# keeffEoghan/tendrils

Measured on AMD Instinct MI355X. Metric: particle-steps/sec (16M particles per GPU), higher is better.
Workload: dtype f32

## Files before the change

tendrils_amd/csrc/th_api.hip:

```cpp
#include "th_ctx.hpp"

using namespace thi;

namespace {

thread_local std::string g_error;

void build_gradient_table(float4 *lut)
{
    for (int a = th::kLutMin; a <= th::kLutMax; ++a) {
        float p = th::permute_ref((float)a);
        float gx, gy, gz;
        th::gradient_ref(p, gx, gy, gz);
        lut[a - th::kLutMin] = make_float4(gx, gy, gz, 0.0f);
    }
}

void options_from_environment(th_options &o)
{
    auto number = [](const char *name, long long otherwise) { const char *e = getenv(name); return e && *e ? atoll(e) : otherwise; };
    o.bucket = (int)number("TH_BUCKET", -1);
    o.resort_steps = (int)number("TH_RESORT_STEPS", 64); if (o.resort_steps <= 0) o.resort_steps = 64;
    o.rebucket_steps = (int)number("TH_REBUCKET_STEPS", 256); if (o.rebucket_steps <= 0) o.rebucket_steps = 256;
    o.fuse = number("TH_FUSE", 1) != 0;
// ... 111 lines not shown

}

extern "C" {

int32_t th_abi_version(void) { return TH_ABI_VERSION; }

const char *th_last_error(void) { return g_error.c_str(); }

th_status th_device_count(int32_t *count)
{
    TH_REQUIRE(count, "null count");
    int n = 0;
    hipError_t e = hipGetDeviceCount(&n);
    if (e != hipSuccess) { *count = 0; return fail(TH_ERR_NO_DEVICE, "hipGetDeviceCount: %s", hipGetErrorString(e)); }
    *count = n;
    return TH_OK;
}

th_status th_create(const th_config *cfg, th_context **out)
{
    TH_REQUIRE(cfg && out, "null argument");
    *out = nullptr;
    TH_REQUIRE(cfg->width > 0 && cfg->height > 0, "state shape must be positive (got %dx%d)", cfg->width, cfg->height);
    TH_REQUIRE(cfg->num_buffers >= 0 && cfg->num_buffers <= 64, "num_buffers out of range");
    TH_REQUIRE(cfg->mode == TH_MODE_EXACT || cfg->mode == TH_MODE_FAST, "unknown mode %d", cfg->mode);
    TH_REQUIRE(cfg->state_format == TH_STATE_F32 || cfg->state_format == TH_STATE_F16, "unknown state format %d", cfg->state_format);
    TH_REQUIRE((uint64_t)cfg->width * (uint64_t)cfg->height < (1ull << 31), "more than 2^31 texels per context");
    int n = 0;
    if (hipGetDeviceCount(&n) != hipSuccess || n <= 0) return fail(TH_ERR_NO_DEVICE, "no HIP device available");
    TH_REQUIRE(cfg->device >= 0 && cfg->device < n, "device %d out of range (have %d)", cfg->device, n);
    hipDeviceProp_t prop;
    TH_HIP(hipGetDeviceProperties(&prop, cfg->device));
    if (strncmp(prop.gcnArchName, "gfx950", 6) != 0)
        return fail(TH_ERR_NO_DEVICE, "device %d is %s; this library ships gfx950 code only", cfg->device, prop.gcnArchName);

    th_context *c = new (std::nothrow) th_context;
    if (!c) return fail(TH_ERR_INVALID, "out of host memory");
    c->cfg = *cfg;
    options_from_environment(c->opt);
    c->packed = cfg->state_format == TH_STATE_F16;
    if (c->cfg.global_height <= 0) c->cfg.global_height = c->cfg.height;
    if (c->cfg.row0 < 0 || c->cfg.row0 + c->cfg.height > c->cfg.global_height) {
        delete c;
        return fail(TH_ERR_INVALID, "row band [%d,%d) outside global height %d", cfg->row0, cfg->row0 + cfg->height, cfg->global_height);
    }
    th_status st = TH_OK;
    auto body = [&]() -> th_status {
        TH_HIP(hipSetDevice(c->cfg.device));
        TH_HIP(hipStreamCreateWithFlags(&c->stream, hipStreamNonBlocking));
        TH_HIP(hipEventCreate(&c->ev0));
        TH_HIP(hipEventCreate(&c->ev1));
        const size_t hv = (size_t)th::hash_table_vectors();
        TH_HIP(hipMalloc((void **)&c->lut_block, (hv + th::kLutSize) * sizeof(float4)));
        c->lut = c->lut_block + hv;
        std::vector<float4> lut(th::kLutSize);
        build_gradient_table(lut.data());
        TH_HIP(hipMemcpy(c->lut, lut.data(), lut.size() * sizeof(float4), hipMemcpyHostToDevice));
        th::launch_hash_tables(c->lut_block, c->stream);
        TH_HIP(hipGetLastError());
        TH_HIP(hipMalloc((void **)&c->d_flag, sizeof(unsigned int)));
        TH_HIP(hipMalloc((void **)&c->partials, th::kStatsBlocks * sizeof(th::StatsPartial)));
        TH_HIP(hipMalloc((void **)&c->d_counters, sizeof(th_counters)));
        TH_HIP(hipMalloc((void **)&c->d_respawned, 2 * sizeof(unsigned long long)));
        TH_HIP(hipMemset(c->d_respawned, 0, 2 * sizeof(unsigned long long)));
        c->fw = c->fh = 1;
        TH_HIP(hipMalloc((void **)&c->flow, sizeof(float4)));
        TH_HIP(hipMemsetAsync(c->flow, 0, sizeof(float4), c->stream));
        TH_HIP(hipMalloc((void **)&c->flow_dec, sizeof(float2)));
        TH_HIP(hipMalloc((void **)&c->targets, c->texels() * sizeof(float4)));
        TH_HIP(hipMemsetAsync(c->targets, 0, c->texels() * sizeof(float4), c->stream));
        for (int k = 0; k < c->cfg.num_buffers; ++k) {
            float4 *b = nullptr;
            if (th_status s = alloc_state(c, &b)) return s;
            c->ring.push_back(b);
        }
        if (th_status s = line_rows(c)) return s;
        TH_HIP(hipStreamSynchronize(c->stream));
        return TH_OK;
    };
    st = body();
    if (st != TH_OK) { std::string keep = g_error; th_destroy(c); g_error = keep; return st; }
    *out = c;
    return TH_OK;
}

th_status th_destroy(th_context *c)
{
    if (!c) return TH_OK;
    (void)hipSetDevice(c->cfg.device);
    if (c->stream) (void)hipStreamSynchronize(c->stream);
    if (c->side) (void)hipStreamSynchronize(c->side);
    if (c->side2) (void)hipStreamSynchronize(c->side2);
    if (c->comm) { (void)c->transport->destroy(c->comm); c->comm = nullptr; }
    (void)hipFree(c->d_status); (void)hipFree(c->own_mem);
    thi::flow_lines_free(c);
    for (float4 *b : c->ring) (void)hipFree(b);
    (void)hipFree(c->flow); (void)hipFree(c->flow_dec); (void)hipFree(c->flow3); (void)hipFree(c->targets); (void)hipFree(c->lut_block);
    (void)hipFree(c->frames[0]); (void)hipFree(c->frames[1]);
    (void)hipFree(c->dep_count); (void)hipFree(c->dep_offset); (void)hipFree(c->dep_blocks); (void)hipFree(c->dep_total);
    (void)hipFree(c->dep_record); (void)hipFree(c->dep_lists); (void)hipFree(c->mrg_keys2); (void)hipFree(c->mrg_colors);
    (void)hipFree(c->bin_mem); (void)hipFree(c->draw_blocks); (void)hipFree(c->draw_block_flags); (void)hipFree(c->d_row_draws); (void)hipFree(c->src_row_index); (void)hipFree(c->src_col_index); (void)hipFree(c->src_slots); (void)hipFree(c->edge_rows); (void)hipFree(c->crowd_mem); (void)hipFree(c->chunk_table);
    (void)hipFree(c->bins_keys); (void)hipFree(c->bins_colors); (void)hipFree(c->crowd_keys); (void)hipFree(c->crowd_sorted); (void)hipFree(c->crowd_parted); (void)hipFree(c->crowd_windows); (void)hipFree(c->gathered);
    if (c->forked) (void)hipEventDestroy(c->forked);
    if (c->joined) (void)hipEventDestroy(c->joined);
    if (c->side) (void)hipStreamDestroy(c->side);
    if (c->joined2) (void)hipEventDestroy(c->joined2);
// ... 397 lines not shown
```

tendrils_amd/csrc/th_kernels.hip:

```cpp
#include "th_kernels.hpp"
#include "th_math.hpp"
#include "th_logic.hpp"

#include <type_traits>
#include <cstdlib>

namespace th {


static int grid_for(size_t n, int blocks_per_cu)
{
    size_t blocks = (n + 255) / 256;
    size_t cap = (size_t)256 * blocks_per_cu;
    return (int)(blocks < cap ? (blocks ? blocks : 1) : cap);
}



__global__ __launch_bounds__(256) void pack_state_kernel(uint2 *dst, const float4 *src, uint32_t n)
{
    for (uint32_t i = blockIdx.x * 256u + threadIdx.x; i < n; i += gridDim.x * 256u) dst[i] = pack_state(src[i]);
}

__global__ __launch_bounds__(256) void unpack_state_kernel(float4 *dst, const uint2 *src, uint32_t n)
{
    for (uint32_t i = blockIdx.x * 256u + threadIdx.x; i < n; i += gridDim.x * 256u) dst[i] = unpack_state(src[i]);
}

void launch_pack_state(void *dst, const float4 *src, uint32_t n, hipStream_t s)
{
    if (n) hipLaunchKernelGGL(pack_state_kernel, dim3(grid_for(n, 8)), dim3(256), 0, s, (uint2 *)dst, src, n);
}

void launch_unpack_state(float4 *dst, const void *src, uint32_t n, hipStream_t s)
{
    if (n) hipLaunchKernelGGL(unpack_state_kernel, dim3(grid_for(n, 8)), dim3(256), 0, s, dst, (const uint2 *)src, n);
}

__global__ __launch_bounds__(256) void hash_tables_kernel(float4 *block)
{
    uint32_t *a = reinterpret_cast<uint32_t *>(block), *b = a + kPermA;
    for (int k = threadIdx.x; k < kPermA; k += 256) a[k] = 4u * (uint32_t)permute_int((float)k);
    for (int k = threadIdx.x; k < kPermB; k += 256) b[k] = 16u * (uint32_t)((int)permute_int((float)k) - kLutMin);
}
void launch_hash_tables(float4 *block, hipStream_t s) { hipLaunchKernelGGL(hash_tables_kernel, dim3(1), dim3(256), 0, s, block); }
int hash_table_vectors() { return kHashVec; }



struct F32Texel {
    using Word = float4;
    static constexpr bool packed = false;
    TH_D static Word empty() { return make_float4(0.0f, 0.0f, 0.0f, 0.0f); }
    TH_D static Word load(const float4 *buf, uint32_t i) { return load_stream(&buf[i]); }
    TH_D static void store(float4 *buf, uint32_t i, Word w) { store_stream(&buf[i], w); }
    TH_D static float4 decode(Word w) { return w; }
    TH_D static Word encode(float4 s) { return s; }
    TH_D static float4 quantize(float4 s) { return s; }
};
struct PackedTexel {
    using Word = v2u;
    static constexpr bool packed = true;
    TH_D static Word empty() { return Word{0x80008000u, 0u}; }
    TH_D static Word load(const float4 *buf, uint32_t i) { return __builtin_nontemporal_load(&reinterpret_cast<const v2u *>(buf)[i]); }
    TH_D static void store(float4 *buf, uint32_t i, Word w) { __builtin_nontemporal_store(w, &reinterpret_cast<v2u *>(buf)[i]); }
    TH_D static float4 decode(Word w) { return unpack_state(make_uint2(w.x, w.y)); }
    TH_D static Word encode(float4 s) { const uint2 q = pack_state(s); return Word{q.x, q.y}; }
    TH_D static float4 quantize(float4 s) { return quantize_state(s); }
};


#define TH_LOGIC_PLAIN_LOOP(Fmt)                                                                                              \
    const float time = p.time_dev ? *p.time_dev : p.u.time;                                                                   \
    __shared__ float4 smem[NOISE ? (PTAB ? kHashVec : 0) + kLutSize : 1];                                                     \
    const float4 *lut = smem + (NOISE && PTAB ? kHashVec : 0);                                                                \
    const HashTables tabs{reinterpret_cast<const uint32_t *>(smem), reinterpret_cast<const uint32_t *>(smem) + kPermA};       \
    if constexpr (NOISE) {                                                                                                    \
        if constexpr (PTAB) fill_hash_tables(smem, p.lut);                                                                    \
        else for (int k = threadIdx.x; k < kLutSize; k += 256) smem[k] = p.lut[k];                                            \
        __syncthreads();                                                                                                      \
    }                                                                                                                         \
    const uint32_t stride = gridDim.x * 256u, end = p.count;                                                                  \
    uint32_t idx = blockIdx.x * 256u + threadIdx.x;                                                                           \
    typename Fmt::Word nxt = Fmt::empty();                                                                                    \
    const uint32_t *perm = p.perm;                                                                                            \
    uint32_t pnxt = idx;                                                                                                      \
    if (idx < end) { nxt = Fmt::load(p.in, idx); if (perm) pnxt = __builtin_nontemporal_load(&perm[idx]); }                   \
    for (; idx < end; idx += stride) {                                                                                        \
        const typename Fmt::Word w = nxt;                                                                                     \
        const uint32_t pid = perm ? pnxt : idx;                                                                               \
        if (idx + stride < end) { nxt = Fmt::load(p.in, idx + stride); if (perm) pnxt = __builtin_nontemporal_load(&perm[idx + stride]); } \
        const float4 st = Fmt::decode(w);                                                                                     \
        const float4 r = integrate<FAST, NOISE, TARGET, POW2, DECODED, NOISE && PTAB>(p, lut, st, pid, time, &tabs);          \
        Fmt::store(p.out, idx, Fmt::encode(r));                                                                               \
        if constexpr (!Fmt::packed) {                                                                                         \
            if (p.seen) {                                                                                                     \
                const bool hidden = (st.x < p.seen_xlo && r.x < p.seen_xlo) || (st.x > p.seen_xhi && r.x > p.seen_xhi) ||     \
                                    (st.y < p.seen_ylo && r.y < p.seen_ylo) || (st.y > p.seen_yhi && r.y > p.seen_yhi);       \
                const unsigned long long any = __ballot(!hidden);                                                             \
                if (__lane_id() == (uint32_t)__builtin_ctzll(__ballot(true))) p.seen[idx >> 6] = any ? 1u : 0u;               \
            }                                                                                                                 \
        }                                                                                                                     \
    }

template <bool FAST, bool NOISE, bool TARGET, bool POW2, bool DECODED, bool PTAB>
__global__ __launch_bounds__(256) void logic_kernel(const LogicParams p) { TH_LOGIC_PLAIN_LOOP(F32Texel) }

template <bool FAST, bool NOISE, bool TARGET, bool POW2, bool DECODED, bool PTAB>
__global__ __launch_bounds__(256) void logic_packed_kernel(const LogicParams p) { TH_LOGIC_PLAIN_LOOP(PackedTexel) }

__global__ __launch_bounds__(256) void logic_generic_kernel(const LogicParams p)
{
    const float time = p.time_dev ? *p.time_dev : p.u.time;
    const uint32_t stride = gridDim.x * 256u;
    for (uint32_t idx = blockIdx.x * 256u + threadIdx.x; idx < p.count; idx += stride) {
        float4 st = p.in[idx];
        uint32_t y = idx / p.width, x = idx - y * p.width;
        p.out[idx] = logic_texel_ref(p, x, y + p.row0, st, idx, time);
// ... 8 lines not shown
    if (b) lift([&](auto... c) { f(std::true_type{}, c...); }, rest...);
    else lift([&](auto... c) { f(std::false_type{}, c...); }, rest...);
}

void launch_logic(const LogicParams &p, const LogicVariant &v, hipStream_t s)
{
    const bool packed = v.format == StateFormat::packed;
    const int grid = packed ? grid_for(p.count, p.perm ? 20 : 8) : grid_for(p.count, 20);
    lift([&](auto fast, auto noise, auto target, auto pow2, auto decoded, auto perm) {
        constexpr bool ptab = noise && perm;
        hipLaunchKernelGGL((packed ? logic_packed_kernel<fast, noise, target, pow2, decoded, ptab>
                                   : logic_kernel<fast, noise, target, pow2, decoded, ptab>), dim3(grid), dim3(256), 0, s, p);
    }, v.mode == TH_MODE_FAST, v.noise, v.target, v.pow2, v.decoded, p.perm != nullptr);
}

void launch_logic_generic(const LogicParams &p, hipStream_t s)
{
    hipLaunchKernelGGL(logic_generic_kernel, dim3(grid_for(p.count, 8)), dim3(256), 0, s, p);
}

TH_D void stats_take(StatsPartial *slot, const float4 &v, float limit, bool first)
{
    const float cap = limit * (1.0f - 9.5367431640625e-07f);
    const bool is_live = v.x != kInert || v.y != kInert;
    const bool is_nan = (v.x != v.x) || (v.y != v.y) || (v.z != v.z) || (v.w != v.w);
    const float sp = __builtin_sqrtf(v.z * v.z + v.w * v.w);
    const bool fin = is_live && !is_nan && sp <= 3.4028234e38f;
    StatsPartial t;
    t.live = __builtin_popcountll(__ballot(is_live)); t.nan = __builtin_popcountll(__ballot(is_nan));
    t.capped = __builtin_popcountll(__ballot(fin && sp >= cap));
    double sum = fin ? (double)sp : 0.0;
    float mx = fin ? sp : 0.0f;
#pragma unroll
    for (int o = 32; o > 0; o >>= 1) {
        sum += __shfl_xor(sum, o);
        const float om = __shfl_xor(mx, o); mx = om > mx ? om : mx;
    }
    if (__lane_id() == (uint32_t)__builtin_ctzll(__ballot(true))) {
        t.sum_speed = sum; t.max_speed = (double)mx;
        if (!first) {
            const StatsPartial o = *slot;
            t.live += o.live; t.nan += o.nan; t.capped += o.capped; t.sum_speed += o.sum_speed;
            t.max_speed = o.max_speed > t.max_speed ? o.max_speed : t.max_speed;
        }
        *slot = t;
    }
}

TH_D void stats_none(StatsPartial *slot, bool first)
{
    if (__ballot(!first) == 0ull && __lane_id() == 0u) *slot = StatsPartial{0ull, 0ull, 0ull, 0.0, 0.0};
}

#define TH_LOGIC_FUSED_LOOP(Fmt)                                                                                              \
    __shared__ float4 smem[NOISE ? kHashVec + kLutSize : 1];                                                                  \
    const float4 *lut = smem + (NOISE ? kHashVec : 0);                                                                        \
    const HashTables tabs{reinterpret_cast<const uint32_t *>(smem), reinterpret_cast<const uint32_t *>(smem) + kPermA};       \
    if constexpr (NOISE) {                                                                                                    \
        fill_hash_tables(smem, p.lut);                                                                                        \
        __syncthreads();                                                                                                      \
    }                                                                                                                         \
    uint32_t idx, stride, end;                                                                                                \
    if constexpr (!BUCKETED) {                                                                                                \
        idx = blockIdx.x * 256u + threadIdx.x;                                                                                \
        stride = gridDim.x * 256u;                                                                                            \
        end = p.count;                                                                                                        \
    } else {                                                                                                                  \
        const uint32_t group = blockIdx.x & 7u, rank = blockIdx.x >> 3, per = (p.count + 7u) >> 3;                            \
        const uint32_t lo = group * per;                                                                                      \
        idx = lo + rank * 256u + threadIdx.x;                                                                                 \
        stride = (gridDim.x >> 3) * 256u;                                                                                     \
        end = lo + per < p.count ? lo + per : p.count;                                                                        \
    }                                                                                                                         \
    typename Fmt::Word nxt = Fmt::empty();                                                                                    \
    uint32_t npid = idx;                                                                                                      \
    [[maybe_unused]] bool first = true;                                                                                       \
    if (idx < end) {                                                                                                          \
        nxt = Fmt::load(p.in, idx);                                                                                           \
        if constexpr (BUCKETED) npid = __builtin_nontemporal_load(&p.perm[idx]);                                              \
    }                                                                                                                         \
    for (; idx < end; idx += stride) {                                                                                        \
        typename Fmt::Word w = nxt, wprev = w;                                                                                \
        const uint32_t pid = BUCKETED ? npid : idx;                                                                           \
        if (idx + stride < end) {                                                                                             \
            nxt = Fmt::load(p.in, idx + stride);                                                                              \
            if constexpr (BUCKETED) npid = __builtin_nontemporal_load(&p.perm[idx + stride]);                                 \
        }                                                                                                                     \
        float4 st = Fmt::decode(w);                                                                                           \
        for (uint32_t k = 0; k < p.nsteps; ++k) {                                                                             \
            if constexpr (!Fmt::packed) wprev = Fmt::encode(st);                                                              \
            else if (k + 1u == p.nsteps && k) wprev = Fmt::encode(st);                                                        \
            st = Fmt::quantize(integrate<FAST, NOISE, TARGET, POW2, false, true, !NOISE>(p, lut, st, pid, p.times[k], &tabs)); \
        }                                                                                                                     \
        if (!Fmt::packed || p.nsteps) w = Fmt::encode(st);                                                                    \
        Fmt::store(p.out_prev, idx, wprev);                                                                                   \
        Fmt::store(p.out, idx, w);                                                                                            \
        if constexpr (STATS) { stats_take(&p.stats_part[blockIdx.x * 4u + (threadIdx.x >> 6)], st, p.u.speedLimit, first); first = false; } \
    }                                                                                                                         \
    if constexpr (STATS) stats_none(&p.stats_part[blockIdx.x * 4u + (threadIdx.x >> 6)], first);

template <bool FAST, bool NOISE, bool TARGET, bool POW2, bool BUCKETED, bool STATS>
__global__ __launch_bounds__(256) void logic_fused_kernel(const LogicParams p) { TH_LOGIC_FUSED_LOOP(F32Texel) }

template <bool FAST, bool NOISE, bool TARGET, bool POW2, bool BUCKETED, bool STATS>
__global__ __launch_bounds__(256, 5) void logic_fused_packed_kernel(const LogicParams p) { TH_LOGIC_FUSED_LOOP(PackedTexel) }

static int fused_grid(uint32_t count, bool bucketed)
{
    const uint32_t blocks = (count + 255u) / 256u;
    const uint32_t grid = bucketed ? 8u * ((((count + 7u) >> 3) + 255u) / 256u) : blocks;
    return (int)(grid ? grid : 1u);
}

void launch_logic_fused(const LogicParams &p, const LogicVariant &v, hipStream_t s)
{
    const bool packed = v.format == StateFormat::packed, bucketed = p.perm != nullptr;
    const int grid = fused_grid(p.count, bucketed);
    lift([&](auto fast, auto noise, auto target, auto pow2, auto bk, auto stats) {
        hipLaunchKernelGGL((packed ? logic_fused_packed_kernel<fast, noise, target, pow2, bk, stats>
                                   : logic_fused_kernel<fast, noise, target, pow2, bk, stats>), dim3(grid), dim3(256), 0, s, p);
    }, v.mode == TH_MODE_FAST, v.noise, v.target, v.pow2, bucketed, p.stats_part != nullptr);
}

TH_D uint32_t tile_key(const TileGeom &g, float px, float py, uint32_t pid)
{
    const uint32_t row = g.row0 + (g.pow2w ? pid >> g.log2w : pid / g.width);
    const uint32_t idle = ((g.row_draws[row >> 5] >> (row & 31u)) & 1u) ^ 1u;
    const bool taps = __builtin_fabsf(px) < __builtin_inff() && __builtin_fabsf(py) < __builtin_inff() &&
                      (px != kInert || py != kInert);
    if (!taps) return 2u * g.ntiles + idle;
    const int tx = (int)__builtin_amdgcn_fmed3f((px * g.view_x + 1.0f) * g.half_fw, 0.0f, g.fwm1);
    const int ty = (int)__builtin_amdgcn_fmed3f((py * g.view_y + 1.0f) * g.half_fh, 0.0f, g.fhm1);
    return 2u * ((uint32_t)(ty >> kTileShift) * g.tiles_x + (uint32_t)(tx >> kTileShift)) + idle;
}

struct WaveRuns { bool head; uint32_t rank, length, head_lane; };
TH_D WaveRuns wave_runs(uint32_t key, bool valid)
{
    const uint32_t lane = __lane_id();
    const uint32_t prev = __shfl_up(key, 1);
    const unsigned long long vmask = __ballot(valid);
    const bool head = valid && (lane == 0 || key != prev);
    const unsigned long long heads = __ballot(head);
    WaveRuns r;
    r.head = head;
    const unsigned long long below = heads & ((2ull << lane) - 1ull);
    r.head_lane = below ? 63u - (uint32_t)__builtin_clzll(below) : 0u;
    r.rank = lane - r.head_lane;
    const unsigned long long above = lane < 63u ? (heads >> (lane + 1u)) : 0ull;
    const uint32_t next = above ? lane + 1u + (uint32_t)__builtin_ctzll(above) : (uint32_t)__builtin_popcountll(vmask);
    r.length = next - lane;
    return r;
}

constexpr uint32_t kBinEmpty = 0xffffffffu;
struct ChunkBins { uint32_t key[kBinSlots], count[kBinSlots], base[kBinSlots]; };

TH_D void bins_clear(ChunkBins &t)
{
    if (threadIdx.x < kBinSlots) { t.key[threadIdx.x] = kBinEmpty; t.count[threadIdx.x] = 0u; t.base[threadIdx.x] = 0u; }
}
TH_D int bins_slot(ChunkBins &t, uint32_t key, bool insert)
{
    uint32_t h = (key * 2654435761u) >> (32 - kBinSlotsLog2);
    for (uint32_t n = 0; n < kBinSlots; ++n, h = (h + 1u) & (kBinSlots - 1u)) {
// ... 731 lines not shown
{
    __shared__ StatsPartial sh[4];
    unsigned long long live = 0, nan = 0, capped = 0;
    double sum = 0.0, mx = 0.0;
    for (int k = threadIdx.x; k < nparts; k += 256) {
        live += part[k].live; nan += part[k].nan; capped += part[k].capped;
        sum += part[k].sum_speed;
        mx = part[k].max_speed > mx ? part[k].max_speed : mx;
    }
#pragma unroll
    for (int o = 32; o > 0; o >>= 1) {
        live += __shfl_xor(live, o); nan += __shfl_xor(nan, o); capped += __shfl_xor(capped, o);
        sum += __shfl_xor(sum, o);
        double om = __shfl_xor(mx, o); mx = om > mx ? om : mx;
    }
    if ((threadIdx.x & 63) == 0) sh[threadIdx.x >> 6] = StatsPartial{live, nan, capped, sum, mx};
    __syncthreads();
    if (threadIdx.x == 0) {
        th_counters c{};
        c.particles = n;
        c.respawned = *respawned;
        for (int w = 0; w < 4; ++w) {
            c.live += sh[w].live; c.nan += sh[w].nan; c.capped += sh[w].capped;
            c.sum_speed += sh[w].sum_speed;
            c.max_speed = sh[w].max_speed > c.max_speed ? sh[w].max_speed : c.max_speed;
        }
        *out = c;
    }
}

__global__ __launch_bounds__(256) void stats_fold_parts_kernel(const StatsPartial *part, uint32_t nparts, StatsPartial *out)
{
    __shared__ StatsPartial sh[4];
    const uint32_t k = blockIdx.x * 256u + threadIdx.x;
    StatsPartial a = k < nparts ? part[k] : StatsPartial{0, 0, 0, 0.0, 0.0};
#pragma unroll
    for (int o = 32; o > 0; o >>= 1) {
        a.live += __shfl_xor(a.live, o); a.nan += __shfl_xor(a.nan, o); a.capped += __shfl_xor(a.capped, o);
        a.sum_speed += __shfl_xor(a.sum_speed, o);
        const double om = __shfl_xor(a.max_speed, o); a.max_speed = om > a.max_speed ? om : a.max_speed;
    }
    if ((threadIdx.x & 63) == 0) sh[threadIdx.x >> 6] = a;
    __syncthreads();
    if (threadIdx.x == 0) {
        StatsPartial t = sh[0];
        for (int w = 1; w < 4; ++w) {
            t.live += sh[w].live; t.nan += sh[w].nan; t.capped += sh[w].capped;
            t.sum_speed += sh[w].sum_speed; t.max_speed = sh[w].max_speed > t.max_speed ? sh[w].max_speed : t.max_speed;
        }
        out[blockIdx.x] = t;
    }
}

uint32_t fused_stats_parts(uint32_t count, bool sorted) { return 4u * (uint32_t)fused_grid(count, sorted); }

void launch_stats_fold(const StatsPartial *parts, uint32_t nparts, StatsPartial *scratch, size_t n, const unsigned long long *respawned,
                       th_counters *out, hipStream_t s)
{
    while (nparts > 4096u) {
        const uint32_t blocks = (nparts + 255u) / 256u;
        hipLaunchKernelGGL(stats_fold_parts_kernel, dim3(blocks), dim3(256), 0, s, parts, nparts, scratch);
        parts = scratch; scratch += blocks; nparts = blocks;
    }
    hipLaunchKernelGGL(stats_fold_kernel, dim3(1), dim3(256), 0, s, parts, (int)nparts, n, respawned, out);
}

void launch_stats(const float4 *state, size_t n, float speed_limit, StatsPartial *partials,
                  const unsigned long long *respawned, th_counters *out, hipStream_t s)
{
    int grid = grid_for(n, 4);
    if (grid > kStatsBlocks) grid = kStatsBlocks;
    hipLaunchKernelGGL(stats_kernel, dim3(grid), dim3(256), 0, s, state, n, speed_limit, partials);
    hipLaunchKernelGGL(stats_fold_kernel, dim3(1), dim3(256), 0, s, partials, grid, n, respawned, out);
}

}
```

tendrils_amd/csrc/th_kernels.hpp:

```cpp
#pragma once
#include <string>

#include <hip/hip_runtime.h>
#include <stdint.h>

#include "../../include/tendrils_hip.h"

namespace th {

constexpr uint32_t kMaxFusedSteps = 32;

constexpr uint32_t kTileChunk = 4096;
constexpr uint32_t kMaxTileBins = 8192;
constexpr uint32_t kSortReplicas = 64;
constexpr uint32_t kBinSlotsLog2 = 6, kBinSlots = 1u << kBinSlotsLog2;

struct TileGeom {
    float view_x, view_y, half_fw, half_fh, fwm1, fhm1;
    uint32_t tiles_x, ntiles;
    uint32_t width, log2w, pow2w, row0;
    const uint32_t *row_draws;
};

struct TileChunk { uint32_t start, count, tile, pad; };
// ... 162 lines not shown
    const unsigned long long *in_keys;
    const float4 *in_colors;
};

struct TrianglePoly {
    int32_t n;
    int32_t x[8], y[8];
};

struct StatsPartial {
    unsigned long long live, nan, capped;
    double sum_speed, max_speed;
};

enum class StateFormat { f32, packed };

struct LogicVariant {
    int32_t mode = TH_MODE_EXACT;
    bool noise = false;
    bool target = false;
    bool pow2 = false;
    bool decoded = false;
    StateFormat format = StateFormat::f32;
    bool operator==(const LogicVariant &o) const
    {
        return mode == o.mode && noise == o.noise && target == o.target && pow2 == o.pow2 && decoded == o.decoded && format == o.format;
    }
};

enum class SortedPass {
    first_sort,
    resort,
    count_in_place,
};

void launch_logic(const LogicParams &p, const LogicVariant &v, hipStream_t stream);
void launch_logic_generic(const LogicParams &p, hipStream_t stream);
void launch_logic_fused(const LogicParams &p, const LogicVariant &v, hipStream_t stream);
inline bool fused_taps_flow3(const LogicVariant &v) { return !v.noise; }
void launch_pack_state(void *dst, const float4 *src, uint32_t n, hipStream_t stream);
void launch_unpack_state(float4 *dst, const void *src, uint32_t n, hipStream_t stream);
void launch_flow_pack3(const float4 *flow, float *xyz, size_t n, hipStream_t stream);
void launch_flow_decode(const float4 *flow, float2 *dec, size_t n, float time, const float *time_dev, float decay,
                        hipStream_t stream);
void launch_logic_sorted(const LogicParams &p, const LogicVariant &v, SortedPass pass, uint32_t max_chunks, hipStream_t stream);
void launch_tile_hist(const TileSortParams &b, hipStream_t stream);
void launch_tile_scan(const TileSortParams &b, hipStream_t stream);
void launch_tile_scatter(const TileSortParams &b, hipStream_t stream);
void launch_unpermute_state(float4 *dst, const float4 *src, const uint32_t *perm, uint32_t n, bool packed, hipStream_t stream);
void launch_permute_state(float4 *dst, const float4 *src, const uint32_t *perm, uint32_t n, bool packed, hipStream_t stream);
void launch_fill(float4 *dst, float4 value, size_t n, hipStream_t stream);
void launch_hash_tables(float4 *block, hipStream_t stream);
int hash_table_vectors();
void launch_finite_check(const float4 *src, size_t n, unsigned int *flag, hipStream_t stream);
void launch_stats_fold(const StatsPartial *parts, uint32_t nparts, StatsPartial *scratch, size_t n, const unsigned long long *respawned,
                       th_counters *out, hipStream_t stream);
uint32_t fused_stats_parts(uint32_t count, bool sorted);
void launch_stats(const float4 *state, size_t n, float speed_limit, StatsPartial *partials, const unsigned long long *respawned,
                  th_counters *out, hipStream_t stream);
void launch_counter_add(unsigned long long *counter, unsigned long long n, hipStream_t s);
void launch_optical_flow(const OpticalFlowParams &p, hipStream_t stream);
uint32_t deposit_scan_words(uint32_t W, uint32_t rows);
size_t deposit_list_words(uint32_t W, uint32_t rows, uint32_t *cap);
void launch_deposit_count(const DepositParams &p, hipStream_t stream);
void launch_deposit_scan(const DepositParams &p, uint32_t *scratch, uint32_t *total, hipStream_t stream);
void launch_deposit_scatter(const DepositParams &p, hipStream_t stream);
int deposit_key_bits(const DepositParams &p);
void launch_export_mark(const DepositParams &p, hipStream_t stream);
void launch_export_write(const DepositParams &p, float *out, hipStream_t stream);
void launch_triangles(const float *positions, int ntri, float view_x, float view_y, float4 color, TrianglePoly *polys,
                      float4 *img, int w, int h, hipStream_t stream);
void launch_deposit_blend(const DepositParams &p, uint32_t total, hipStream_t stream);
void launch_view_fill(uchar4 *view, size_t texels, float4 color, hipStream_t stream);
void launch_view_copy(uchar4 *view, const uchar4 *src, size_t texels, hipStream_t stream);
constexpr int kBinShift = 4;
constexpr uint32_t kBinCap = 4096;
constexpr uint32_t kBinReplicas = 16;
constexpr uint32_t kBinPage = 256;
constexpr uint32_t kBinFirstPages = 128;
constexpr uint32_t kBinPagesLimit = 4096;
constexpr int32_t kBinsMaxExtent = 4096;
enum { kTotFragments = 0, kTotOob = 1, kTotFlags = 2, kTotLarge = 3, kTotGiant = 4, kTotLong = 5, kTotPool = 6, kTotCrowdKeys = 7, kTotWindows = 8, kTotWords = 12 };
enum { kBinsPoolExhausted = 1u, kBinsBoundBroken = 2u, kBinsBinFull = 4u, kBinsWaitBroken = 8u };
void launch_bins_block_list(const DepositParams &p, uint8_t *flags, uint32_t *list, uint32_t *count, uint32_t *src_slots, hipStream_t stream);
void launch_bins_edge_rows(const DepositParams &p, float4 *rows, hipStream_t stream);
void launch_bins_fused(const DepositParams &p, hipStream_t stream);
void launch_bins_owner_counts(const DepositParams &p, const OwnerParams &o, hipStream_t stream);
void launch_bins_owner_extract(const DepositParams &p, const OwnerParams &o, hipStream_t stream);
void launch_bins_owner_insert(const DepositParams &p, const OwnerParams &o, hipStream_t stream);
void launch_bins_regroup(const DepositParams &p, hipStream_t stream);
void launch_bins_part_giants(const DepositParams &p, hipStream_t stream);
void launch_bins_blend_giants(const DepositParams &p, hipStream_t stream);
void launch_bins_sort_long(const DepositParams &p, hipStream_t stream);
void launch_bins_walk_long(const DepositParams &p, hipStream_t stream);
void launch_bins_blend_crowd(const DepositParams &p, hipStream_t stream);
void launch_bins_blend(const DepositParams &p, hipStream_t stream);
size_t crowd_words_per_bin();
struct Transport {
    const char *name;
    int (*destroy)(void *comm);
    int (*allreduce_counters)(void *comm, void *counters_dev, hipStream_t stream);
    int (*allgather_bytes)(void *comm, const void *send, void *recv, const size_t *bytes, const size_t *offset, int rank, int world, hipStream_t stream);
    int (*alltoallv)(void *comm, const void *send, const size_t *send_counts, const size_t *send_off, void *recv, const size_t *recv_counts,
                     const size_t *recv_off, size_t elem, int world, hipStream_t stream);
    int (*allreduce_max_u32)(void *comm, uint32_t *word_dev, hipStream_t stream);
};
// ... 35 lines not shown
```

tendrils_amd/csrc/th_logic.hpp:

```cpp
#pragma once
#include "th_kernels.hpp"
#include "th_math.hpp"

namespace th {

typedef float v4f __attribute__((ext_vector_type(4)));
typedef unsigned v2u __attribute__((ext_vector_type(2)));
typedef float v2f __attribute__((ext_vector_type(2)));

TH_D uint32_t mad_u24_s(uint32_t a, uint32_t b, uint32_t c)
{
    uint32_t r;
    asm("v_mad_u32_u24 %0, %1, %2, %3" : "=v"(r) : "v"(a), "s"(b), "v"(c));
    return r;
}

TH_D float4 load_stream(const float4 *p)
{
    v4f v = __builtin_nontemporal_load(reinterpret_cast<const v4f *>(p));
    return make_float4(v.x, v.y, v.z, v.w);
}
TH_D void store_stream(float4 *p, float4 a)
{
    v4f v = {a.x, a.y, a.z, a.w};
// ... 51 lines not shown
    float fcx = (float)x + 0.5f, fcy = (float)y_global + 0.5f;
    float uvx = fcx / p.wf, uvy = fcy / p.hf;
    float posx = st.x, posy = st.y, velx = st.z, vely = st.w;
    if (!(posx != kInert || posy != kInert)) return st;

    float i = (fcx + (fcy * p.wf)) / (p.wf * p.hf);
    float nscale = vary(u.noiseScale, i, u.varyNoiseScale);
    float nx = posx * nscale, ny = posy * nscale;
    float ntime = time * vary(u.noiseSpeed, i, u.varyNoiseSpeed);
    float wx = snoise_ref(nx, ny, uvx + ntime);
    float wy = snoise_ref(nx, ny, uvy + ntime + 1234.5678f);

    float sx = posx * u.viewSize[0], sy = posy * u.viewSize[1];
    float fu = 0.0f + (1.0f * (sx + 1.0f)) / 2.0f;
    float fv = 0.0f + (1.0f * (sy + 1.0f)) / 2.0f;
    int tx = (int)__builtin_amdgcn_fmed3f(th_floor(fu * p.fwf), 0.0f, p.fwm1);
    int ty = (int)__builtin_amdgcn_fmed3f(th_floor(fv * p.fhf), 0.0f, p.fhm1);
    float4 ft = p.flow[(size_t)ty * p.fw + tx];
    float k = __builtin_fmaxf(0.0f, 1.0f - ((time - ft.z) * u.flowDecay));
    float ffx = (0.0f + ft.x * k * 1.0f) / 1.0f, ffy = (0.0f + ft.y * k * 1.0f) / 1.0f;

    float vfw = vary(u.forceWeight, i, u.varyForce);
    float vflw = vary(u.flowWeight, i, u.varyFlow);
    float vnw = vary(u.noiseWeight, i, u.varyNoise);
    float nvx = (velx * u.damping * u.dt) + (vfw * ((ffx * u.dt * vflw) + (wx * u.dt * vnw)));
    float nvy = (vely * u.damping * u.dt) + (vfw * ((ffy * u.dt * vflw) + (wy * u.dt * vnw)));

    float4 tg = p.targets[local_index];
    float vtg = vary(u.target, i, u.varyTarget);
    nvx += (tg.x - posx) * vtg;
    nvy += (tg.y - posy) * vtg;

    float speed = __builtin_sqrtf(nvx * nvx + nvy * nvy);
    float r = __builtin_fminf(speed, u.speedLimit) / speed;
    nvx *= r; nvy *= r;
    return make_float4(posx + nvx, posy + nvy, nvx, nvy);
}

struct NoiseCorners {
    float ax, ay, az, bx, by, bz, cx, cy, cz, dx, dy, dz;
    int j0, j1, j2, j3;
};

constexpr int kPermA = 292, kPermB = 584;
constexpr int kHashVec = (kPermA + kPermB) / 4;
struct HashTables {
    const uint32_t *permA, *permB;
};

TH_D void fill_hash_tables(float4 *smem, const float4 *lut_global)
{
    const float4 *block = lut_global - kHashVec;
    for (int k = threadIdx.x; k < kHashVec + kLutSize; k += 256) smem[k] = block[k];
}


template <bool FAST>
TH_D NoiseCorners snoise_corners_tab(float vx, float vy, float vz, float sxy, const HashTables &T)
{
    NoiseCorners n;
    float s = mad<FAST>(vz, kC3, sxy);
    float ix = th_floor(vx + s), iy = th_floor(vy + s), iz = th_floor(vz + s);
    float t = mad<FAST>(iz, kC6, mad<FAST>(iy, kC6, ix * kC6));
    float ax = (vx - ix) + t, ay = (vy - iy) + t, az = (vz - iz) + t;

    const float ax1 = ax - 1.0f, ay1 = ay - 1.0f, az1 = az - 1.0f;
    float bx, by, bz, cx, cy, cz;
    uint32_t e1x, e2x, e1y, e2y;
    unsigned long long mz1, mz2;
    {
        unsigned long long l1, l2, l3, m;
        asm("v_cmp_lt_f32 %[l1], %[ax], %[ay]\n\t"
            "v_cmp_lt_f32 %[l2], %[ay], %[az]\n\t"
            "v_cmp_lt_f32 %[l3], %[az], %[ax]\n\t"
            "s_andn2_b64 %[m], %[l3], %[l1]\n\t"     "v_cndmask_b32 %[bx], %[ax], %[ax1], %[m]\n\t"   "v_cndmask_b32 %[e1x], 0, 16, %[m]\n\t"
            "s_andn2_b64 %[m], %[l1], %[l2]\n\t"     "v_cndmask_b32 %[by], %[ay], %[ay1], %[m]\n\t"   "v_cndmask_b32 %[e1y], 0, 4, %[m]\n\t"
            "s_andn2_b64 %[mz1], %[l2], %[l3]\n\t"   "v_cndmask_b32 %[bz], %[az], %[az1], %[mz1]\n\t"
            "s_orn2_b64 %[m], %[l3], %[l1]\n\t"      "v_cndmask_b32 %[cx], %[ax], %[ax1], %[m]\n\t"   "v_cndmask_b32 %[e2x], 0, 16, %[m]\n\t"
            "s_orn2_b64 %[m], %[l1], %[l2]\n\t"      "v_cndmask_b32 %[cy], %[ay], %[ay1], %[m]\n\t"   "v_cndmask_b32 %[e2y], 0, 4, %[m]\n\t"
            "s_orn2_b64 %[mz2], %[l2], %[l3]\n\t"    "v_cndmask_b32 %[cz], %[az], %[az1], %[mz2]"
            : [l1] "=&s"(l1), [l2] "=&s"(l2), [l3] "=&s"(l3), [m] "=&s"(m), [mz1] "=&s"(mz1), [mz2] "=&s"(mz2),
              [bx] "=&v"(bx), [by] "=&v"(by), [bz] "=&v"(bz), [cx] "=&v"(cx), [cy] "=&v"(cy), [cz] "=&v"(cz),
              [e1x] "=&v"(e1x), [e2x] "=&v"(e2x), [e1y] "=&v"(e1y), [e2y] "=&v"(e2y)
            : [ax] "v"(ax), [ay] "v"(ay), [az] "v"(az), [ax1] "v"(ax1), [ay1] "v"(ay1), [az1] "v"(az1)
            : "scc");
    }
    n.ax = ax; n.ay = ay; n.az = az;
    n.bx = bx + kC6; n.by = by + kC6; n.bz = bz + kC6;
    n.cx = cx + kC3; n.cy = cy + kC3; n.cz = cz + kC3;
    n.dx = ax - 0.5f; n.dy = ay - 0.5f; n.dz = az - 0.5f;

    const uint32_t xi = (uint32_t)mod289_int(ix), yi = (uint32_t)mod289_int(iy), zi = (uint32_t)mod289_int(iz);
    const uint32_t *pa = reinterpret_cast<const uint32_t *>(reinterpret_cast<const char *>(T.permA) + (zi << 2));
    const uint32_t pz0 = pa[0], pz1 = pa[1];
    uint32_t sel1, sel2;
    asm("v_cndmask_b32 %0, %2, %3, %4\n\tv_cndmask_b32 %1, %2, %3, %5"
        : "=&v"(sel1), "=&v"(sel2) : "v"(pz0), "v"(pz1), "s"(mz1), "s"(mz2));
    const uint32_t y4 = yi << 2;
    auto stage_y = [&](uint32_t off) { return *reinterpret_cast<const uint32_t *>(reinterpret_cast<const char *>(T.permB) + off); };
    const uint32_t q0 = stage_y(pz0 + y4), q1 = stage_y(sel1 + y4 + e1y), q2 = stage_y(sel2 + y4 + e2y),
                   q3 = stage_y(pz1 + y4 + 4u);
    const uint32_t x16 = xi << 4;
    n.j0 = (int)(q0 + x16); n.j1 = (int)(q1 + x16 + e1x); n.j2 = (int)(q2 + x16 + e2x); n.j3 = (int)(q3 + x16 + 16u);
    return n;
}

// ... 201 lines not shown
```

Measured before the change: 197.2 billion.

## Restructure fused logic kernel into paired chunks with async global-to-LDS prefetch

Replaces the grid-stride loop in the fused logic kernel with a fixed schedule. Each workgroup handles one or two 256-particle chunks, and the grid is sized so that most groups take two chunks while a tail of single-chunk groups balances the last rounds. The second chunk's state and permutation, along with the hash/gradient tables, are prefetched using direct global-to-LDS loads (global_load_lds) so they overlap with the first chunk's integration. The intent is to remove the register-held prefetch and to cut launch-tail imbalance. In exchange it pads the LUT block to a multiple of 64 vectors, uses more LDS per block, lays out stats partials per chunk, and adds optional timestamp instrumentation behind a macro.

```diff
diff --git a/tendrils_amd/csrc/th_api.hip b/tendrils_amd/csrc/th_api.hip
--- a/tendrils_amd/csrc/th_api.hip
+++ b/tendrils_amd/csrc/th_api.hip
@@ -187,7 +187,7 @@
         TH_HIP(hipEventCreate(&c->ev0));
         TH_HIP(hipEventCreate(&c->ev1));
         const size_t hv = (size_t)th::hash_table_vectors();
-        TH_HIP(hipMalloc((void **)&c->lut_block, (hv + th::kLutSize) * sizeof(float4)));
+        TH_HIP(hipMalloc((void **)&c->lut_block, (size_t)th::lut_block_vectors() * sizeof(float4)));
         c->lut = c->lut_block + hv;
         std::vector<float4> lut(th::kLutSize);
         build_gradient_table(lut.data());
diff --git a/tendrils_amd/csrc/th_kernels.hip b/tendrils_amd/csrc/th_kernels.hip
--- a/tendrils_amd/csrc/th_kernels.hip
+++ b/tendrils_amd/csrc/th_kernels.hip
@@ -42,9 +42,11 @@
     uint32_t *a = reinterpret_cast<uint32_t *>(block), *b = a + kPermA;
     for (int k = threadIdx.x; k < kPermA; k += 256) a[k] = 4u * (uint32_t)permute_int((float)k);
     for (int k = threadIdx.x; k < kPermB; k += 256) b[k] = 16u * (uint32_t)((int)permute_int((float)k) - kLutMin);
+    for (int k = kHashVec + kLutSize + threadIdx.x; k < kLutBlockVec; k += 256) block[k] = make_float4(0.0f, 0.0f, 0.0f, 0.0f);
 }
 void launch_hash_tables(float4 *block, hipStream_t s) { hipLaunchKernelGGL(hash_tables_kernel, dim3(1), dim3(256), 0, s, block); }
 int hash_table_vectors() { return kHashVec; }
+int lut_block_vectors() { return kLutBlockVec; }
 
 
 
@@ -54,6 +56,8 @@
     TH_D static Word empty() { return make_float4(0.0f, 0.0f, 0.0f, 0.0f); }
     TH_D static Word load(const float4 *buf, uint32_t i) { return load_stream(&buf[i]); }
     TH_D static void store(float4 *buf, uint32_t i, Word w) { store_stream(&buf[i], w); }
+    TH_D static void load_lds(uint32_t *lds, const float4 *buf, uint32_t i) { load_to_lds16_stream(&buf[i], lds + 4u * (threadIdx.x & ~63u)); }
+    TH_D static Word from_lds(const uint32_t *lds) { return *reinterpret_cast<const float4 *>(lds + 4u * threadIdx.x); }
     TH_D static float4 decode(Word w) { return w; }
     TH_D static Word encode(float4 s) { return s; }
     TH_D static float4 quantize(float4 s) { return s; }
@@ -64,6 +68,13 @@
     TH_D static Word empty() { return Word{0x80008000u, 0u}; }
     TH_D static Word load(const float4 *buf, uint32_t i) { return __builtin_nontemporal_load(&reinterpret_cast<const v2u *>(buf)[i]); }
     TH_D static void store(float4 *buf, uint32_t i, Word w) { __builtin_nontemporal_store(w, &reinterpret_cast<v2u *>(buf)[i]); }
+    TH_D static void load_lds(uint32_t *lds, const float4 *buf, uint32_t i)
+    {
+        const uint32_t *src = reinterpret_cast<const uint32_t *>(buf) + 2u * (size_t)i;
+        load_to_lds4_stream(src, lds + (threadIdx.x & ~63u));
+        load_to_lds4_stream(src + 1, lds + 256u + (threadIdx.x & ~63u));
+    }
+    TH_D static Word from_lds(const uint32_t *lds) { return Word{lds[threadIdx.x], lds[256u + threadIdx.x]}; }
     TH_D static float4 decode(Word w) { return unpack_state(make_uint2(w.x, w.y)); }
     TH_D static Word encode(float4 s) { const uint2 q = pack_state(s); return Word{q.x, q.y}; }
     TH_D static float4 quantize(float4 s) { return quantize_state(s); }
@@ -178,52 +189,82 @@
     if (__ballot(!first) == 0ull && __lane_id() == 0u) *slot = StatsPartial{0ull, 0ull, 0ull, 0.0, 0.0};
 }
 
+#ifdef TH_FUSED_STAMPS
+constexpr uint32_t kStampWaves = 1u << 18, kStampWords = 10u;
+__device__ unsigned long long g_fused_stamps[kStampWaves * kStampWords];
+TH_D void fused_stamp(uint32_t k)
+{
+    const uint32_t wave = blockIdx.x * 4u + (threadIdx.x >> 6);
+    if (wave < kStampWaves && __lane_id() == 0u) g_fused_stamps[wave * kStampWords + k] = __builtin_amdgcn_s_memtime();
+}
+TH_D void fused_stamp_where()
+{
+    const uint32_t wave = blockIdx.x * 4u + (threadIdx.x >> 6);
+    const unsigned long long hw = __builtin_amdgcn_s_getreg((31 << 11) | 4), xcc = __builtin_amdgcn_s_getreg((3 << 11) | 20);
+    if (wave < kStampWaves && __lane_id() == 0u) g_fused_stamps[wave * kStampWords + 8u] = hw | xcc << 32;
+}
+#define TH_FUSED_STAMP(k) fused_stamp(k)
+#define TH_FUSED_STAMP_WHERE() fused_stamp_where()
+#else
+#define TH_FUSED_STAMP(k) do {} while (0)
+#define TH_FUSED_STAMP_WHERE() do {} while (0)
+#endif
+
 #define TH_LOGIC_FUSED_LOOP(Fmt)                                                                                              \
-    __shared__ float4 smem[NOISE ? kHashVec + kLutSize : 1];                                                                  \
+    TH_FUSED_STAMP(0); TH_FUSED_STAMP_WHERE();                                                                                \
+    __shared__ float4 smem[NOISE ? kLutBlockVec : 1];                                                                         \
+    __shared__ __attribute__((aligned(16))) uint32_t next_state[256u * sizeof(typename Fmt::Word) / 4u];                      \
+    __shared__ uint32_t next_pid[BUCKETED ? 256 : 1];                                                                         \
     const float4 *lut = smem + (NOISE ? kHashVec : 0);                                                                        \
     const HashTables tabs{reinterpret_cast<const uint32_t *>(smem), reinterpret_cast<const uint32_t *>(smem) + kPermA};       \
-    if constexpr (NOISE) {                                                                                                    \
-        fill_hash_tables(smem, p.lut);                                                                                        \
-        __syncthreads();                                                                                                      \
+    constexpr uint32_t groups = BUCKETED ? 8u : 1u;                                                                           \
+    const uint32_t group = blockIdx.x % groups, q = blockIdx.x / groups, per = BUCKETED ? (p.count + 7u) >> 3 : p.count;      \
+    const uint32_t lo = group * per, end = lo + per < p.count ? lo + per : p.count;                                           \
+    const uint32_t chunks = (per + 255u) >> 8, wgs = gridDim.x / groups, pairs = chunks > wgs ? chunks - wgs : 0u;            \
+    const bool pair = q < pairs;                                                                                              \
+    const uint32_t rank = pair ? 2u * q : q + pairs, last = p.count - 1u;                                                  \
+    uint32_t idx = lo + rank * 256u + threadIdx.x;                                                                            \
+    const uint32_t at = idx < last ? idx : last;                                                                              \
+    typename Fmt::Word w = Fmt::load(p.in, at);                                                                               \
+    uint32_t pid = idx;                                                                                                       \
+    if constexpr (BUCKETED) pid = __builtin_nontemporal_load(&p.perm[at]);                                                    \
+    if constexpr (NOISE) fill_hash_tables_lds(smem, p.lut);                                                                   \
+    if (pair) {                                                                                                               \
+        const uint32_t atb = idx + 256u < last ? idx + 256u : last;                                                           \
+        Fmt::load_lds(next_state, p.in, atb);                                                                                 \
+        if constexpr (BUCKETED) load_to_lds4_stream(&p.perm[atb], next_pid + (threadIdx.x & ~63u));                          \
     }                                                                                                                         \
-    uint32_t idx, stride, end;                                                                                                \
-    if constexpr (!BUCKETED) {                                                                                                \
-        idx = blockIdx.x * 256u + threadIdx.x;                                                                                \
-        stride = gridDim.x * 256u;                                                                                            \
-        end = p.count;                                                                                                        \
-    } else {                                                                                                                  \
-        const uint32_t group = blockIdx.x & 7u, rank = blockIdx.x >> 3, per = (p.count + 7u) >> 3;                            \
-        const uint32_t lo = group * per;                                                                                      \
-        idx = lo + rank * 256u + threadIdx.x;                                                                                 \
-        stride = (gridDim.x >> 3) * 256u;                                                                                     \
-        end = lo + per < p.count ? lo + per : p.count;                                                                        \
-    }                                                                                                                         \
-    typename Fmt::Word nxt = Fmt::empty();                                                                                    \
-    uint32_t npid = idx;                                                                                                      \
-    [[maybe_unused]] bool first = true;                                                                                       \
-    if (idx < end) {                                                                                                          \
-        nxt = Fmt::load(p.in, idx);                                                                                           \
-        if constexpr (BUCKETED) npid = __builtin_nontemporal_load(&p.perm[idx]);                                              \
-    }                                                                                                                         \
-    for (; idx < end; idx += stride) {                                                                                        \
-        typename Fmt::Word w = nxt, wprev = w;                                                                                \
-        const uint32_t pid = BUCKETED ? npid : idx;                                                                           \
-        if (idx + stride < end) {                                                                                             \
-            nxt = Fmt::load(p.in, idx + stride);                                                                              \
-            if constexpr (BUCKETED) npid = __builtin_nontemporal_load(&p.perm[idx + stride]);                                 \
+    wait_lds_loads();                                                                                                         \
+    __syncthreads();                                                                                                          \
+    TH_FUSED_STAMP(1);                                                                                                        \
+    _Pragma("nounroll")                                                                                                       \
+    for (uint32_t chunk = 0;; ++chunk) {                                                                                      \
+        [[maybe_unused]] StatsPartial *part = nullptr;                                                                        \
+        if constexpr (STATS) part = &p.stats_part[((rank + chunk) * groups + group) * 4u + (threadIdx.x >> 6)];               \
+        [[maybe_unused]] bool took = false;                                                                                   \
+        if (idx < end) {                                                                                                      \
+            typename Fmt::Word wprev = w;                                                                                     \
+            float4 st = Fmt::decode(w);                                                                                       \
+            TH_FUSED_STAMP(2u + 3u * chunk);                                                                                  \
+            for (uint32_t k = 0; k < p.nsteps; ++k) {                                                                         \
+                if constexpr (!Fmt::packed) wprev = Fmt::encode(st);                                                          \
+                else if (k + 1u == p.nsteps && k) wprev = Fmt::encode(st);                                                    \
+                st = Fmt::quantize(integrate<FAST, NOISE, TARGET, POW2, false, true, !NOISE>(p, lut, st, pid, p.times[k], &tabs)); \
+            }                                                                                                                 \
+            TH_FUSED_STAMP(3u + 3u * chunk);                                                                                  \
+            if (!Fmt::packed || p.nsteps) w = Fmt::encode(st);                                                                \
+            Fmt::store(p.out_prev, idx, wprev);                                                                               \
+            Fmt::store(p.out, idx, w);                                                                                        \
+            if constexpr (STATS) { stats_take(part, st, p.u.speedLimit, true); took = true; }                                 \
         }                                                                                                                     \
-        float4 st = Fmt::decode(w);                                                                                           \
-        for (uint32_t k = 0; k < p.nsteps; ++k) {                                                                             \
-            if constexpr (!Fmt::packed) wprev = Fmt::encode(st);                                                              \
-            else if (k + 1u == p.nsteps && k) wprev = Fmt::encode(st);                                                        \
-            st = Fmt::quantize(integrate<FAST, NOISE, TARGET, POW2, false, true, !NOISE>(p, lut, st, pid, p.times[k], &tabs)); \
-        }                                                                                                                     \
-        if (!Fmt::packed || p.nsteps) w = Fmt::encode(st);                                                                    \
-        Fmt::store(p.out_prev, idx, wprev);                                                                                   \
-        Fmt::store(p.out, idx, w);                                                                                            \
-        if constexpr (STATS) { stats_take(&p.stats_part[blockIdx.x * 4u + (threadIdx.x >> 6)], st, p.u.speedLimit, first); first = false; } \
-    }                                                                                                                         \
-    if constexpr (STATS) stats_none(&p.stats_part[blockIdx.x * 4u + (threadIdx.x >> 6)], first);
+                                         \
+        if constexpr (STATS) stats_none(part, !took);                                                                         \
+        TH_FUSED_STAMP(4u + 3u * chunk);                                                                                      \
+        if (chunk || !pair) break;                                                                                            \
+        idx += 256u;                                                                                                          \
+        w = Fmt::from_lds(next_state);                                                                                        \
+        pid = BUCKETED ? next_pid[threadIdx.x] : idx;                                                                         \
+    }
 
 template <bool FAST, bool NOISE, bool TARGET, bool POW2, bool BUCKETED, bool STATS>
 __global__ __launch_bounds__(256) void logic_fused_kernel(const LogicParams p) { TH_LOGIC_FUSED_LOOP(F32Texel) }
@@ -231,12 +272,30 @@
 template <bool FAST, bool NOISE, bool TARGET, bool POW2, bool BUCKETED, bool STATS>
 __global__ __launch_bounds__(256, 5) void logic_fused_packed_kernel(const LogicParams p) { TH_LOGIC_FUSED_LOOP(PackedTexel) }
 
+#ifndef TH_FUSED_TAIL_ROUNDS
+#define TH_FUSED_TAIL_ROUNDS 2
+#endif
+constexpr uint32_t kFusedTailRounds = TH_FUSED_TAIL_ROUNDS;
+static uint32_t fused_chunks(uint32_t count, bool bucketed) { return ((bucketed ? (count + 7u) >> 3 : count) + 255u) / 256u; }
 static int fused_grid(uint32_t count, bool bucketed)
 {
-    const uint32_t blocks = (count + 255u) / 256u;
-    const uint32_t grid = bucketed ? 8u * ((((count + 7u) >> 3) + 255u) / 256u) : blocks;
+    const uint32_t groups = bucketed ? 8u : 1u, chunks = fused_chunks(count, bucketed);
+    const uint64_t tail = (uint64_t)kFusedTailRounds * 6u * 256u / groups;
+    uint32_t single = chunks < tail ? chunks : (uint32_t)tail;
+    single += (chunks - single) & 1u;
+    const uint32_t grid = groups * ((chunks - single) / 2u + single);
     return (int)(grid ? grid : 1u);
 }
+
+#ifdef TH_FUSED_STAMPS
+extern "C" int th_debug_fused_stamps(unsigned long long *out, uint32_t waves)
+{
+    const size_t bytes = (size_t)(waves < kStampWaves ? waves : kStampWaves) * kStampWords * sizeof(unsigned long long);
+    if (hipMemcpyFromSymbol(out, HIP_SYMBOL(g_fused_stamps), bytes) != hipSuccess) return 1;
+    void *dev = nullptr;
+    return hipGetSymbolAddress(&dev, HIP_SYMBOL(g_fused_stamps)) != hipSuccess || hipMemset(dev, 0, bytes) != hipSuccess;
+}
+#endif
 
 void launch_logic_fused(const LogicParams &p, const LogicVariant &v, hipStream_t s)
 {
@@ -1074,7 +1133,11 @@
     }
 }
 
-uint32_t fused_stats_parts(uint32_t count, bool sorted) { return 4u * (uint32_t)fused_grid(count, sorted); }
+uint32_t fused_stats_parts(uint32_t count, bool sorted)
+{
+    const uint32_t chunks = (sorted ? 8u : 1u) * fused_chunks(count, sorted);
+    return 4u * (chunks ? chunks : 1u);
+}
 
 void launch_stats_fold(const StatsPartial *parts, uint32_t nparts, StatsPartial *scratch, size_t n, const unsigned long long *respawned,
                        th_counters *out, hipStream_t s)
diff --git a/tendrils_amd/csrc/th_kernels.hpp b/tendrils_amd/csrc/th_kernels.hpp
--- a/tendrils_amd/csrc/th_kernels.hpp
+++ b/tendrils_amd/csrc/th_kernels.hpp
@@ -238,6 +238,7 @@
 void launch_fill(float4 *dst, float4 value, size_t n, hipStream_t stream);
 void launch_hash_tables(float4 *block, hipStream_t stream);
 int hash_table_vectors();
+int lut_block_vectors();
 void launch_finite_check(const float4 *src, size_t n, unsigned int *flag, hipStream_t stream);
 void launch_stats_fold(const StatsPartial *parts, uint32_t nparts, StatsPartial *scratch, size_t n, const unsigned long long *respawned,
                        th_counters *out, hipStream_t stream);
diff --git a/tendrils_amd/csrc/th_logic.hpp b/tendrils_amd/csrc/th_logic.hpp
--- a/tendrils_amd/csrc/th_logic.hpp
+++ b/tendrils_amd/csrc/th_logic.hpp
@@ -127,6 +127,26 @@
 {
     const float4 *block = lut_global - kHashVec;
     for (int k = threadIdx.x; k < kHashVec + kLutSize; k += 256) smem[k] = block[k];
+}
+
+#define TH_LDS_LOAD(name, bytes, aux)                                                                                   \
+    TH_D void name(const void *src, void *lds_wave_base)                                                                \
+    {                                                                                                                   \
+        __builtin_amdgcn_global_load_lds((const __attribute__((address_space(1))) void *)src,                           \
+                                         (__attribute__((address_space(3))) void *)lds_wave_base, bytes, 0, aux);       \
+    }
+TH_LDS_LOAD(load_to_lds16, 16, 0)
+TH_LDS_LOAD(load_to_lds16_stream, 16, 2)
+TH_LDS_LOAD(load_to_lds4_stream, 4, 2)
+#undef TH_LDS_LOAD
+TH_D void wait_lds_loads() { asm volatile("s_waitcnt vmcnt(0)" ::: "memory"); }
+
+constexpr int kLutBlockVec = (kHashVec + kLutSize + 63) / 64 * 64;
+TH_D void fill_hash_tables_lds(float4 *smem, const float4 *lut_global)
+{
+    const float4 *block = lut_global - kHashVec;
+#pragma unroll
+    for (int k = threadIdx.x; k < kLutBlockVec; k += 256) load_to_lds16(&block[k], smem + (k & ~63));
 }
 
 
```

Result: no change. 196.9 billion (-0.2%).
